# nju-ee/MODE-2022

Hardware: AMD Instinct MI355X
Metric: ERP stereo pairs/sec (512x1024, 192 disp) fwd+bwd (higher is better)
Workload: dtype fp32 storage/accumulate; products: 2xfp16 split (22-bit, per-tensor 2^k scale, 3 MFMAs) in the stride-1 3x3x3 / spherical / 3x3 layers incl. gradients (DESIGN 3u/3v); 3xbf16 split (24-bit, 6 MFMAs) in the stride-2 / transposed 3x3x3 layers and the polar spherical tiles (3j-3l); fp32 MFMA in the 32->; 1 GPU; ModeDisparity(192,Sphere,1024x512 Cassini) fwd+bwd+Adam step, batch 2/GPU (BASELINE configs[2]); global_batch=2, conv_arith=bf16x6, init=recipe state, seed 1 (tests/golden/recipe.py), parallelism=dp1

## Files before the change

mode-2022_amd/csrc/classif_head.hip:

```cpp
#include "bn_internal.h"
#include "conv3d_internal.h"

#include <algorithm>

namespace {

typedef float f32x16 __attribute__((ext_vector_type(16)));
constexpr int NT = 256;

__device__ __forceinline__ f32x16 mfma32(float a, float b, f32x16 c) { return __builtin_amdgcn_mfma_f32_32x32x2f32(a, b, c, 0, 0, 0); }

constexpr int ZTH = 16, ZIH = ZTH + 2, ZIW = 34, ZPL = ZIH * ZIW;
constexpr int ZDC = 12;
static_assert(ZIH + 2 == 4 * 5, "18 row groups + 36 halo-column positions in 2 groups = 5 groups per wave");

template <bool BNRELU, bool C32>
__global__ __launch_bounds__(NT, 2) void classif_fwd_kernel(const float* __restrict__ x, const float* __restrict__ w,
                                                            const float* __restrict__ scale, const float* __restrict__ shift,
                                                            const float* __restrict__ add, float* __restrict__ y, int B, int Ci, int D,
                                                            int H, int W, int nDc, int nHt, int nWt) {
  extern __shared__ __attribute__((aligned(16))) float zl[];
  float2* coefl = reinterpret_cast<float2*>(zl + 27 * ZPL);
  int t = xcd_remap(blockIdx.x, gridDim.x);
  const int wt = t % nWt;
  t /= nWt;
  const int ht = t % nHt;
  t /= nHt;
  const int dc = t % nDc;
  const int b = t / nDc;
  const int w0 = wt * 32, h0 = ht * ZTH, dlo = dc * ZDC, dhi = min(D, dlo + ZDC);
  const int tid = threadIdx.x, wave = tid >> 6, lane = tid & 63;
  const int j = lane & 31, kh = lane >> 5;
  const long long HW = (long long)H * W, DHW = (long long)D * HW;
  const float* xb = x + (long long)b * Ci * DHW;

  if (BNRELU && tid < 32) coefl[tid] = tid < Ci ? make_float2(scale[tid], shift[tid]) : make_float2(0.f, 0.f);
  float a0[16];
#pragma unroll
  for (int ks = 0; ks < 16; ++ks) {
    const int c = ks + 16 * kh;
    a0[ks] = (j < 27 && c < Ci) ? w[min(c, Ci - 1) * 27 + min(j, 26)] : 0.f;
  }
  int poff[5], pz[5];
  bool pok[5];
#pragma unroll
  for (int g5 = 0; g5 < 5; ++g5) {
    const int g = wave * 5 + g5;
    int row, gw, zc;
    bool in = true;
    if (g < ZIH) {
      row = g;
      gw = w0 + j;
      zc = 1 + j;
    } else {
      const int p = (g - ZIH) * 32 + j;
      in = p < 2 * ZIH;
      row = in ? p >> 1 : 0;
      gw = (p & 1) ? w0 + 32 : w0 - 1;
      zc = (p & 1) ? 33 : 0;
    }
    const int gh = h0 + row - 1;
    pok[g5] = in && gh >= 0 && gh < H && gw >= 0 && gw < W;
    poff[g5] = pok[g5] ? gh * W + gw : 0;
    pz[g5] = in ? row * ZIW + zc : -1;
  }
  if (C32) {
#pragma unroll
    for (int g5 = 0; g5 < 5; ++g5) poff[g5] += (int)((unsigned)(16 * kh) * (unsigned)DHW);
  }
  const int wx = tid & 31, hq = tid >> 5;
  float om1[2] = {0.f, 0.f}, o0[2] = {0.f, 0.f};

  float bv[5][16];
  auto load_group = [&](int dz, int g5) {
    const float* xp = xb + (long long)dz * HW;
    if (C32) {
      const unsigned pbyte = (unsigned)poff[g5] << 2;
#pragma unroll
      for (int ks = 0; ks < 16; ++ks)
        bv[g5][ks] = *reinterpret_cast<const float*>(reinterpret_cast<const char*>(xp + (long long)ks * DHW) + pbyte);
    } else {
      unsigned dhw = (unsigned)DHW;
      asm volatile("" : "+s"(dhw));
#pragma unroll
      for (int ks = 0; ks < 16; ++ks) bv[g5][ks] = xp[(unsigned)poff[g5] + (unsigned)min(ks + 16 * kh, Ci - 1) * dhw];
    }
  };
  const int dstart = max(dlo - 1, 0), dend = min(dhi, D - 1);
#pragma unroll
  for (int g5 = 0; g5 < 5; ++g5) load_group(dstart, g5);
  __syncthreads();
  const int gwx = w0 + wx;
  long long oidx[2];
  bool ook[2];
#pragma unroll
  for (int o = 0; o < 2; ++o) {
    const int gh = h0 + hq + 8 * o;
    ook[o] = gh < H && gwx < W;
    oidx[o] = ook[o] ? (long long)b * DHW + (long long)gh * W + gwx : 0;
  }

  for (int dz = dstart; dz <= dend; ++dz) {
    float s[3][2];
    const int dout = dz - 1;
    float addv[2] = {0.f, 0.f};
    if (add) {
#pragma unroll
      for (int o = 0; o < 2; ++o) addv[o] = add[oidx[o] + (long long)max(dout, 0) * HW];
    }
    f32x16 acc[5];
    int co = 16 * kh;
    const int dnext = min(dz + 1, dend);
#pragma unroll
    for (int g5 = 0; g5 < 5; ++g5) {
      asm volatile("" : "+v"(co));
      acc[g5] = (f32x16){0};
#pragma unroll
      for (int ks = 0; ks < 16; ++ks) {
        if (BNRELU) {
          const float2 cf = coefl[co + ks];
          float a = __builtin_fmaf(bv[g5][ks], cf.x, cf.y);
          asm("" : "+v"(a));
          acc[g5] = mfma32(a0[ks], pok[g5] ? relu_nan(a) : 0.f, acc[g5]);
        } else {
          acc[g5] = mfma32(a0[ks], pok[g5] ? bv[g5][ks] : 0.f, acc[g5]);
        }
      }
      __builtin_amdgcn_sched_barrier(0);
      load_group(dnext, g5);
      __builtin_amdgcn_sched_barrier(0);
    }
#pragma unroll
    for (int g5 = 0; g5 < 5; ++g5) {
      if (pz[g5] >= 0) {
#pragma unroll
        for (int q = 0; q < 16; ++q) {
          const int i = (q & 3) + 8 * (q >> 2) + 4 * kh;
          if (i < 27) zl[i * ZPL + pz[g5]] = acc[g5][q];
        }
      }
    }
    __syncthreads();
#pragma unroll
    for (int o = 0; o < 2; ++o) {
      const float* zp = zl + (hq + 8 * o) * ZIW + wx;
#pragma unroll
      for (int kd = 0; kd < 3; ++kd) {
        float v = 0.f;
#pragma unroll
        for (int k9 = 0; k9 < 9; ++k9) {
          v += zp[(kd * 9 + k9) * ZPL + (k9 / 3) * ZIW + (k9 % 3)];
          asm volatile("" : "+v"(v));
        }
        s[kd][o] = v;
      }
    }
    __syncthreads();
#pragma unroll
    for (int o = 0; o < 2; ++o) {
      if (dout >= dlo && ook[o]) y[oidx[o] + (long long)dout * HW] = om1[o] + s[2][o] + addv[o];
      om1[o] = o0[o] + s[1][o];
      o0[o] = s[0][o];
    }
  }
  if (dend < dhi) {
#pragma unroll
    for (int o = 0; o < 2; ++o) {
      if (ook[o]) {
        const long long idx = oidx[o] + (long long)dend * HW;
        y[idx] = add ? om1[o] + add[idx] : om1[o];
      }
    }
  }
}

constexpr int GTH = 8;
constexpr int XS = GTH * 32 + 1;
constexpr int GH = GTH + 2, GW = 34, GPL = GH * GW;

__global__ __launch_bounds__(NT) void classif_bww_kernel(const float* __restrict__ gy, const float* __restrict__ x,
                                                         const float* __restrict__ mean, const float* __restrict__ scale,
                                                         const float* __restrict__ shift, float* __restrict__ part, int B, int Ci, int D,
                                                         int H, int W, int nHt, int nWt, int T, int S) {
  __shared__ __attribute__((aligned(16))) float xl[32 * XS];
  __shared__ float gl[3 * GPL];
  const int s = blockIdx.x;
  const int tid = threadIdx.x, wave = tid >> 6, lane = tid & 63;
  const int hwv = tid >> 5, l32 = tid & 31;
  const long long HW = (long long)H * W, DHW = (long long)D * HW;
  const int j = lane & 31;
  const int tap = j < 27 ? j : 0;
  const int toff = (2 - tap / 9) * GPL + (2 - (tap / 3) % 3) * GW + (2 - tap % 3);
  const float mu = j < Ci ? mean[j] : 0.f, sc = j < Ci ? scale[j] : 0.f, sh = j < Ci ? shift[j] : 0.f;
  const float nanv = __builtin_nanf("");
  f32x16 accq = {0}, accm = {0};

  for (int tt = s; tt < T; tt += S) {
    int t = tt;
    const int wt = t % nWt;
    t /= nWt;
    const int ht = t % nHt;
    t /= nHt;
    const int d0 = t % D;
    const int b = t / D;
    const int w0 = wt * 32, h0 = ht * GTH;
    const float* xb = x + (long long)b * Ci * DHW + d0 * HW;
    const float* gb = gy + (long long)b * DHW;
#pragma unroll 1
    for (int kb = 0; kb < 256; kb += 64) {
      float t8[8];
#pragma unroll
      for (int jj = 0; jj < 8; ++jj) {
        const int r = kb + jj * 8 + hwv;
        const int c = r >> 3, gh = h0 + (r & 7), gw = w0 + l32;
        const bool ok = c < Ci && gh < H && gw < W;
        const float v = xb[ok ? c * DHW + (long long)gh * W + gw : 0];
        t8[jj] = ok ? v : nanv;
      }
#pragma unroll
      for (int jj = 0; jj < 8; ++jj) {
        const int r = kb + jj * 8 + hwv;
        xl[(r >> 3) * XS + (r & 7) * 32 + l32] = t8[jj];
      }
    }
    for (int idx = tid; idx < 3 * GPL; idx += NT) {
      const int zz = idx / GPL, rem = idx - zz * GPL;
      const int yy = rem / GW, xx = rem - yy * GW;
      const int gd = d0 - 1 + zz, gh = h0 - 1 + yy, gw = w0 - 1 + xx;
      const bool ok = gd >= 0 && gd < D && gh >= 0 && gh < H && gw >= 0 && gw < W;
      const float v = gb[ok ? gd * HW + (long long)gh * W + gw : 0];
      gl[idx] = ok ? v : 0.f;
    }
    __syncthreads();
    const float* ap = xl + (lane & 31) * XS + (lane >> 5);
    const float* bp = gl + toff + (lane >> 5);
#pragma unroll
    for (int rr = 0; rr < 2; ++rr) {
      const int row = wave * 2 + rr;
#pragma unroll 8
      for (int ks = 0; ks < 16; ++ks) {
        const float yv = ap[row * 32 + 2 * ks], gv = bp[row * GW + 2 * ks];
        const bool m = __builtin_fmaf(yv, sc, sh) > 0.f;
        accq = mfma32(m ? yv - mu : 0.f, gv, accq);
        accm = mfma32(m ? 1.f : 0.f, gv, accm);
      }
    }
    __syncthreads();
  }
  float* red = xl;
#pragma unroll
  for (int q = 0; q < 16; ++q) {
    const int i = (q & 3) + 8 * (q >> 2) + 4 * (lane >> 5);
    red[wave * 1024 + i * 32 + (lane & 31)] = accq[q];
    red[4096 + wave * 1024 + i * 32 + (lane & 31)] = accm[q];
  }
  __syncthreads();
  float* pb = part + (long long)s * 2048;
  for (int idx = tid; idx < 2048; idx += NT) {
    const float* r = red + (idx >> 10) * 4096 + (idx & 1023);
    float lo = r[0] + r[1024], hi = r[2048] + r[3072];
    asm volatile("" : "+v"(lo), "+v"(hi));
    pb[idx] = lo + hi;
  }
}

constexpr int XS2 = 260;

template <int TC>
__global__ __launch_bounds__(NT) void classif_bww2_kernel(const float* __restrict__ gy, const float* __restrict__ x,
                                                          const float* __restrict__ mean, const float* __restrict__ scale,
                                                          const float* __restrict__ shift, float* __restrict__ part, int B, int Ci, int D,
                                                          int H, int W, int nHt, int nWt, int T, int S) {
  constexpr int TR = 256 / TC, GWD = TC + 2, GHT = TR + 2, GPL2 = GHT * GWD, NG = (3 * GPL2 + NT - 1) / NT;
  __shared__ __attribute__((aligned(16))) float xl[32 * XS2];
  __shared__ float gl[3 * GPL2];
  const int s = blockIdx.x;
  const int tid = threadIdx.x, wave = tid >> 6, lane = tid & 63;
  const long long HW = (long long)H * W, DHW = (long long)D * HW;
  const int j = lane & 31, khalf = lane >> 5;
  const int tap = j < 27 ? j : 0;
  const int toff = (2 - tap / 9) * GPL2 + (2 - (tap / 3) % 3) * GWD + (2 - tap % 3);
  const float mu = j < Ci ? mean[j] : 0.f, sc = j < Ci ? scale[j] : 0.f, sh = j < Ci ? shift[j] : 0.f;
  const float nanv = __builtin_nanf("");
  f32x16 accq = {0}, accm = {0};

  const int v0 = 4 * (tid & 63), srow = v0 / TC, scol = v0 % TC;
  float4 px[8];
  float pg[NG];
  unsigned pxok = 0, pgok = 0;
  auto request = [&](int tt) {
    int t = tt;
    const int wt = t % nWt;
    t /= nWt;
    const int ht = t % nHt;
    t /= nHt;
    const int d0 = t % D;
    const int b = t / D;
    const int w0 = wt * TC, h0 = ht * TR;
    const float* xb = x + (long long)b * Ci * DHW + d0 * HW;
    const float* gb = gy + (long long)b * DHW;
    const int gh = h0 + srow, gw = w0 + scol;
    const unsigned vok = (unsigned)(gh < H) & (unsigned)(gw < W);
    const long long voff = (long long)vok * ((long long)gh * W + gw);
    pxok = 0;
#pragma unroll
    for (int i = 0; i < 8; ++i) {
      const int c = (tid >> 6) + 4 * i;
      px[i] = *reinterpret_cast<const float4*>(xb + (long long)min(c, Ci - 1) * DHW + voff);
      pxok |= (vok & (unsigned)(c < Ci)) << i;
    }
    pgok = 0;
#pragma unroll
    for (int i = 0; i < NG; ++i) {
      const int idx = min(tid + NT * i, 3 * GPL2 - 1);
      const int zz = idx / GPL2, rem = idx - zz * GPL2;
      const int yy = rem / GWD, xx = rem - yy * GWD;
      const int gd = d0 - 1 + zz, gh2 = h0 - 1 + yy, gw2 = w0 - 1 + xx;
      const unsigned ok = (unsigned)(gd >= 0) & (unsigned)(gd < D) & (unsigned)(gh2 >= 0) & (unsigned)(gh2 < H) & (unsigned)(gw2 >= 0) &
                          (unsigned)(gw2 < W);
      pg[i] = gb[(long long)ok * (gd * HW + (long long)gh2 * W + gw2)];
      pgok |= ok << i;
    }
  };
  if (s < T) request(s);
  asm volatile("s_waitcnt vmcnt(0)" ::: "memory");

  for (int tt = s; tt < T; tt += S) {
    __syncthreads();
#pragma unroll
    for (int i = 0; i < 8; ++i) {
      const int c = (tid >> 6) + 4 * i;
      const bool ok = (pxok >> i) & 1;
      *reinterpret_cast<float4*>(xl + c * XS2 + v0) = ok ? px[i] : make_float4(nanv, nanv, nanv, nanv);
    }
#pragma unroll
    for (int i = 0; i < NG; ++i)
      if (tid + NT * i < 3 * GPL2) gl[tid + NT * i] = ((pgok >> i) & 1) ? pg[i] : 0.f;
    __syncthreads();
    request(tt + S < T ? tt + S : tt);
    __builtin_amdgcn_sched_barrier(0);
    const float* ap = xl + j * XS2 + wave * 64 + 4 * khalf;
#pragma unroll
    for (int m = 0; m < 8; ++m) {
      const float4 a4 = *reinterpret_cast<const float4*>(ap + 8 * m);
      const int v = wave * 64 + 8 * m;
      const float* bp = gl + toff + (v / TC) * GWD + (v % TC) + 4 * khalf;
      const float ye[4] = {a4.x, a4.y, a4.z, a4.w};
#pragma unroll
      for (int e = 0; e < 4; ++e) {
        const float gv = bp[e];
        const bool mk = __builtin_fmaf(ye[e], sc, sh) > 0.f;
        accq = mfma32(mk ? ye[e] - mu : 0.f, gv, accq);
        accm = mfma32(mk ? 1.f : 0.f, gv, accm);
      }
    }
  }
  __syncthreads();
  float* red = xl;
#pragma unroll
  for (int q = 0; q < 16; ++q) {
    const int i = (q & 3) + 8 * (q >> 2) + 4 * khalf;
    red[wave * 1024 + i * 32 + j] = accq[q];
    red[4096 + wave * 1024 + i * 32 + j] = accm[q];
  }
  __syncthreads();
  float* pb = part + (long long)s * 2048;
  for (int idx = tid; idx < 2048; idx += NT) {
    const float* r = red + (idx >> 10) * 4096 + (idx & 1023);
    float lo = r[0] + r[1024], hi = r[2048] + r[3072];
    asm volatile("" : "+v"(lo), "+v"(hi));
    pb[idx] = lo + hi;
  }
}

__global__ __launch_bounds__(NT) void classif_bwd_reduce_kernel(const float* __restrict__ part, const float* __restrict__ w,
                                                                const float* __restrict__ gamma, const float* __restrict__ beta,
                                                                const float* __restrict__ mean, const float* __restrict__ invstd,
                                                                const float* __restrict__ scale, float* __restrict__ gw,
                                                                float* __restrict__ ggamma, float* __restrict__ gbeta,
                                                                float4* __restrict__ coef, int S, double count, int accumulate) {
  __shared__ double qs[27], ms[27];
  const int c = blockIdx.x, wave = threadIdx.x >> 6, lane = threadIdx.x & 63;
  for (int t = wave; t < 27; t += NT / 64) {
    const float* p = part + c * 32 + t;
    double q = 0.0, m = 0.0;
    for (int s = lane; s < S; s += 64) {
      q += (double)p[(long long)s * 2048];
      m += (double)p[(long long)s * 2048 + 1024];
    }
#pragma unroll
    for (int off = 32; off > 0; off >>= 1) {
      q += __shfl_xor(q, off, 64);
      m += __shfl_xor(m, off, 64);
    }
    if (lane == 0) {
      qs[t] = q;
      ms[t] = m;
    }
  }
  __syncthreads();
  if (threadIdx.x < 27) {
    const int t = threadIdx.x;
    const float v = (float)((double)scale[c] * qs[t] + (double)beta[c] * ms[t]);
    gw[c * 27 + t] = accumulate ? gw[c * 27 + t] + v : v;
  }
  if (threadIdx.x == 0) {
    double sgy = 0.0, sg = 0.0;
    for (int t = 0; t < 27; ++t) {
      sgy += (double)w[c * 27 + t] * qs[t];
      sg += (double)w[c * 27 + t] * ms[t];
    }
    const double is = invstd[c], mu = mean[c], gm = gamma[c];
    const double dgamma = is * sgy;
    const double A = gm * is;
    coef[c] = make_float4((float)A, (float)(-A * is * dgamma / count), (float)(A * (mu * is * dgamma - sg) / count), 0.f);
    if (accumulate) {
      ggamma[c] += (float)dgamma;
      gbeta[c] += (float)sg;
    } else {
      ggamma[c] = (float)dgamma;
      gbeta[c] = (float)sg;
    }
  }
}

constexpr int BTD = 2, BTH = 8;
constexpr int BID = BTD + 2, BIH = BTH + 2, BIW = 34;

__global__ __launch_bounds__(NT) void classif_bwd_apply_kernel(const float* __restrict__ gy, const float* __restrict__ w,
                                                               const float* __restrict__ y, const float* __restrict__ scale,
                                                               const float* __restrict__ shift, const float4* __restrict__ coef,
                                                               float* __restrict__ gx, int B, int Ci, int D, int H, int W, int nDt,
                                                               int nHt, int nWt) {
  __shared__ float tile[BID * BIH * BIW];
  __shared__ __attribute__((aligned(16))) float ctab[32 * 8];
  int t = xcd_remap(blockIdx.x, gridDim.x);
  const int wt = t % nWt;
  t /= nWt;
  const int ht = t % nHt;
  t /= nHt;
  const int dt = t % nDt;
  const int b = t / nDt;
  const int w0 = wt * 32, h0 = ht * BTH, d0 = dt * BTD;
  const int tid = threadIdx.x, wave = tid >> 6, lane = tid & 63;
  const long long HW = (long long)H * W, DHW = (long long)D * HW;
  const float* gb = gy + (long long)b * DHW;

  for (int idx = tid; idx < BID * BIH * BIW; idx += NT) {
    const int dz = idx / (BIH * BIW), rem = idx - dz * (BIH * BIW);
    const int hy = rem / BIW, wx = rem - hy * BIW;
    const int gd = d0 + dz - 1, gh = h0 + hy - 1, gw = w0 + wx - 1;
    const bool ok = gd >= 0 && gd < D && gh >= 0 && gh < H && gw >= 0 && gw < W;
    const float v = gb[ok ? gd * HW + gh * W + gw : 0];
    tile[idx] = ok ? v : 0.f;
  }
  if (tid < 32) {
    const int c = tid < Ci ? tid : Ci - 1;
    const float4 k = coef[c];
    ctab[tid * 8 + 0] = scale[c];
    ctab[tid * 8 + 1] = shift[c];
    ctab[tid * 8 + 2] = k.x;
    ctab[tid * 8 + 3] = k.y;
    ctab[tid * 8 + 4] = k.z;
  }
  float a[14];
  int toff[14];
  const int c = lane & 31;
#pragma unroll
  for (int ks = 0; ks < 14; ++ks) {
    const int k = 2 * ks + (lane >> 5);
    a[ks] = (k < 27 && c < Ci) ? w[c * 27 + 26 - k] : 0.f;
    const int kk = k < 27 ? k : 26;
    toff[ks] = (kk / 9) * (BIH * BIW) + ((kk / 3) % 3) * BIW + kk % 3;
  }
  const int gw = w0 + (lane & 31);
  long long sp[4];
  bool rok[4];
#pragma unroll
  for (int r = 0; r < 4; ++r) {
    const int row = wave * 4 + r;
    const int gd = d0 + row / BTH, gh = h0 + row % BTH;
    rok[r] = gd < D && gh < H && gw < W;
    sp[r] = rok[r] ? gd * HW + (long long)gh * W + gw : 0;
  }
  __syncthreads();

  f32x16 acc[4];
#pragma unroll
  for (int r = 0; r < 4; ++r) acc[r] = (f32x16){0};
  const float* tp = tile + (lane & 31);
#pragma unroll
  for (int ks = 0; ks < 14; ++ks)
#pragma unroll
    for (int r = 0; r < 4; ++r) {
      const int row = wave * 4 + r;
      acc[r] = mfma32(a[ks], tp[(row / BTH) * (BIH * BIW) + (row % BTH) * BIW + toff[ks]], acc[r]);
    }

  const float* yb = y + (long long)b * Ci * DHW;
  float* gxb = gx + (long long)b * Ci * DHW;
#pragma unroll
  for (int q = 0; q < 16; ++q) {
    const int i = (q & 3) + 8 * (q >> 2) + 4 * (lane >> 5);
    const int ic = i < Ci ? i : Ci - 1;
    const float4 k0 = *reinterpret_cast<const float4*>(ctab + ic * 8);
    const float Cc = ctab[ic * 8 + 4];
    float yv[4];
// ... 266 lines not shown
```

mode-2022_amd/csrc/conv1x1.hip:

```cpp
#include "common.h"

namespace {

typedef float f32x16 __attribute__((ext_vector_type(16)));
constexpr int NT = 256;

__device__ __forceinline__ f32x16 mfma32(float a, float b, f32x16 c) {
  return __builtin_amdgcn_mfma_f32_32x32x2f32(a, b, c, 0, 0, 0);
}

struct P1 {
  int B, K, rows;
  int H, W, Ho, Wo;
  int s;
  int NK4;
  int MT;
};

__global__ void pack_w1(const float* __restrict__ w, float* __restrict__ wp, int rows, int K, int MT, int NK4, int flip, int fold,
                        mode_bn_epilogue bn) {
  const long long total = (long long)MT * NK4 * 64 * 4;
  if (fold && blockIdx.x == 0)
    for (int o = threadIdx.x; o < rows; o += blockDim.x) wp[total + o] = fold_shift(bn, o);
  for (long long idx = (long long)blockIdx.x * blockDim.x + threadIdx.x; idx < total; idx += (long long)gridDim.x * blockDim.x) {
    const int j = (int)(idx & 3);
    const int lane = (int)((idx >> 2) & 63);
    const long long r = idx >> 8;
    const int k4 = (int)(r % NK4), mt = (int)(r / NK4);
    const int o = mt * 32 + (lane & 31), c = 8 * k4 + 2 * j + (lane >> 5);
    float v = 0.f;
    if (o < rows && c < K) v = flip ? w[(long long)c * rows + o] : w[(long long)o * K + c];
    if (fold && o < rows) v *= fold_scale(bn, o);
    wp[idx] = v;
  }
}

template <int MTB, bool EPI, bool SCATTER>
__global__ __launch_bounds__(NT) void conv1x1_kernel(const float* __restrict__ x, const float4* __restrict__ wp, float* __restrict__ y,
                                                     P1 d, Epi epi) {
  const int wave = threadIdx.x >> 6, lane = threadIdx.x & 63;
  const int No = d.Ho * d.Wo;
  const int tpi = (No + 31) / 32;
  const long long tile = (long long)blockIdx.x * 4 + wave;
  if (tile >= (long long)d.B * tpi) return;
  const int b = (int)(tile / tpi);
  const int q = (int)(tile % tpi) * 32 + (lane & 31);
  const bool ok = q < No;
  const int ho = q / d.Wo, wo = q - ho * d.Wo;
  const long long kplane = SCATTER ? (long long)No : (long long)d.H * d.W;
  const long long koff = !ok ? 0 : (SCATTER ? (long long)q : (long long)ho * d.s * d.W + (long long)wo * d.s);
  const float* xb = x + (long long)b * d.K * kplane + koff;
  const int half = lane >> 5;
  const int mt0 = blockIdx.y * MTB;

  f32x16 acc[MTB];
#pragma unroll
  for (int m = 0; m < MTB; ++m) acc[m] = (f32x16){0};
  const float4* wq = wp + ((long long)mt0 * d.NK4) * 64 + lane;
  const int kmax = d.K - 1;

  float bv[4];
  float4 av[MTB];
  auto load = [&](int k4, float (&b4)[4], float4 (&a4)[MTB]) {
#pragma unroll
    for (int j = 0; j < 4; ++j) {
      const int c = min(8 * k4 + 2 * j + half, kmax);
      b4[j] = xb[(long long)c * kplane];
    }
#pragma unroll
    for (int m = 0; m < MTB; ++m) a4[m] = (mt0 + m < d.MT) ? wq[((long long)m * d.NK4 + k4) * 64] : make_float4(0.f, 0.f, 0.f, 0.f);
  };
  load(0, bv, av);
  for (int k4 = 0; k4 < d.NK4; ++k4) {
    float bn_[4];
    float4 an_[MTB];
    if (k4 + 1 < d.NK4) load(k4 + 1, bn_, an_);
    __builtin_amdgcn_sched_barrier(0);
#pragma unroll
    for (int j = 0; j < 4; ++j)
#pragma unroll
      for (int m = 0; m < MTB; ++m) {
        const float a = j == 0 ? av[m].x : j == 1 ? av[m].y : j == 2 ? av[m].z : av[m].w;
        acc[m] = mfma32(a, bv[j], acc[m]);
      }
    if (k4 + 1 < d.NK4) {
#pragma unroll
      for (int j = 0; j < 4; ++j) bv[j] = bn_[j];
#pragma unroll
      for (int m = 0; m < MTB; ++m) av[m] = an_[m];
    }
  }

  if (!ok) return;
  const long long oplane = SCATTER ? (long long)d.H * d.W : (long long)No;
  const long long ooff = SCATTER ? (long long)ho * d.s * d.W + (long long)wo * d.s : (long long)q;
  float* yb = y + (long long)b * d.rows * oplane + ooff;
#pragma unroll
  for (int m = 0; m < MTB; ++m)
#pragma unroll
    for (int r = 0; r < 16; ++r) {
      const int o = (mt0 + m) * 32 + (r & 3) + 8 * (r >> 2) + 4 * half;
      if (o < d.rows) {
        const long long idx = (long long)o * oplane;
        yb[idx] = EPI ? apply_epi(epi, acc[m][r], o, (yb - y) + idx) : acc[m][r];
      }
    }
}

template <bool EPI, bool SCATTER>
int launch1(const float* x, const float* wpack, float* y, const P1& d, hipStream_t st, const Epi& epi, const char* who) {
  const long long tiles = (long long)d.B * mode::cdiv(d.Ho * d.Wo, 32);
  const int gx = mode::cdiv(tiles, 4);
  const float4* wp4 = reinterpret_cast<const float4*>(wpack);
  if (d.MT == 1)
    hipLaunchKernelGGL((conv1x1_kernel<1, EPI, SCATTER>), dim3(gx, 1), dim3(NT), 0, st, x, wp4, y, d, epi);
  else if (d.MT == 2)
    hipLaunchKernelGGL((conv1x1_kernel<2, EPI, SCATTER>), dim3(gx, 1), dim3(NT), 0, st, x, wp4, y, d, epi);
  else
    hipLaunchKernelGGL((conv1x1_kernel<4, EPI, SCATTER>), dim3(gx, mode::cdiv(d.MT, 4)), dim3(NT), 0, st, x, wp4, y, d, epi);
  return mode::check_launch(who);
}

int check1(const void* a, const void* b, const void* c, const void* wp, int B, int Ci, int H, int W, int Co, int stride, const char* who) {
  MODE_REQUIRE(B >= 0 && Ci > 0 && Co > 0 && H > 0 && W > 0, MODE_ERR_BAD_ARG, "%s: non-positive size", who);
  MODE_REQUIRE(stride == 1 || stride == 2, MODE_ERR_UNSUPPORTED, "%s: stride %d not implemented (1 or 2)", who, stride);
  MODE_REQUIRE((long long)std::max(Ci, Co) * H * W < (1ll << 31), MODE_ERR_UNSUPPORTED, "%s: a sample larger than 2^31 elements", who);
  if (B == 0) return MODE_OK;
  MODE_REQUIRE(a && b && c && wp, MODE_ERR_BAD_ARG, "%s: null pointer", who);
  return MODE_OK;
}

int fwd1(const float* x, const float* w, float* y, float* wpack, int B, int Ci, int H, int W, int Co, int stride, hipStream_t st,
         const mode_bn_epilogue* bn, const char* who) {
  P1 d;
  d.B = B; d.K = Ci; d.rows = Co; d.H = H; d.W = W; d.s = stride;
  d.Ho = (H - 1) / stride + 1; d.Wo = (W - 1) / stride + 1;
  d.NK4 = mode::cdiv(Ci, 8); d.MT = mode::cdiv(Co, 32);
  const long long npack = (long long)d.MT * d.NK4 * 256;
  if (mode::pack_needed()) hipLaunchKernelGGL(pack_w1, dim3(mode::cdiv(npack, 256)), dim3(256), 0, st, w, wpack, Co, Ci, d.MT, d.NK4, 0, bn ? 1 : 0,
                     bn ? *bn : mode_bn_epilogue());
  const Epi epi = make_epi(bn, wpack + npack);
  return bn ? launch1<true, false>(x, wpack, y, d, st, epi, who) : launch1<false, false>(x, wpack, y, d, st, epi, who);
}

struct W1 {
  int B, Ci, Co, H, W, Ho, Wo, s;
  int groups;
  int S;
};

constexpr int BW_PX = 64;
constexpr int BW_PITCH = BW_PX + 1;
constexpr int BW_TILE = 128 * BW_PITCH;
constexpr int BW_LDS_FLOATS = 2 * BW_TILE > 3 * 4 * 1024 ? 2 * BW_TILE : 3 * 4 * 1024;

template <int S2>
__global__ __launch_bounds__(NT) void conv1x1_bww_kernel(const float* __restrict__ gy, const float* __restrict__ x, float* __restrict__ part,
                                                         W1 d) {
  extern __shared__ __attribute__((aligned(16))) float sm[];
  const int wave = threadIdx.x >> 6, lane = threadIdx.x & 63;
  const int row = lane & 31, half = lane >> 5;
  const int o0 = blockIdx.y * 64, c0 = blockIdx.z * 64;
  const long long No = (long long)d.Ho * d.Wo, HW = (long long)d.H * d.W;
  const int tiles_img = (int)((No + BW_PX - 1) / BW_PX);
  const long long total = (long long)d.B * tiles_img;
  const long long per = (total + d.S - 1) / d.S;
  const long long t_lo = (long long)blockIdx.x * per, t_hi = min(total, t_lo + per);

  const int sr = threadIdx.x >> 4, sp = (threadIdx.x & 15) * 4;
  float4 v[8];
  auto issue = [&](long long t) {
    const int b = (int)(t / tiles_img);
    const long long q = (t % tiles_img) * BW_PX + sp;
    const bool ok = q < No;
#pragma unroll
    for (int u = 0; u < 8; ++u) {
      const int r = sr + 16 * u;
      if (r < 64) {
        const int o = o0 + r;
        v[u] = *reinterpret_cast<const float4*>(gy + ((long long)b * d.Co + (o < d.Co ? o : 0)) * No + (ok ? q : 0));
        if (!ok || o >= d.Co) v[u] = make_float4(0.f, 0.f, 0.f, 0.f);
      } else {
        const int c = c0 + r - 64;
        const float* xr = x + ((long long)b * d.Ci + (c < d.Ci ? c : 0)) * HW;
        if (S2 == 1) {
          v[u] = *reinterpret_cast<const float4*>(xr + (ok ? q : 0));
        } else {
          const int ho = (int)((ok ? q : 0) / d.Wo), wo = (int)((ok ? q : 0) - (long long)ho * d.Wo);
          const float* p = xr + (long long)ho * 2 * d.W + 2 * wo;
          const float4 u0 = *reinterpret_cast<const float4*>(p), u1 = *reinterpret_cast<const float4*>(p + 4);
          v[u] = make_float4(u0.x, u0.z, u1.x, u1.z);
        }
        if (!ok || c >= d.Ci) v[u] = make_float4(0.f, 0.f, 0.f, 0.f);
      }
    }
  };
  auto commit = [&](float* buf) {
#pragma unroll
    for (int u = 0; u < 8; ++u) {
      float* p = buf + (sr + 16 * u) * BW_PITCH + sp;
      p[0] = v[u].x;
      p[1] = v[u].y;
      p[2] = v[u].z;
      p[3] = v[u].w;
    }
  };

  f32x16 acc[2][2];
#pragma unroll
  for (int i = 0; i < 4; ++i) acc[i >> 1][i & 1] = (f32x16){0};
  if (t_lo < t_hi) {
    issue(t_lo);
    commit(sm);
  }
  __syncthreads();
  int buf = 0;
  for (long long t = t_lo; t < t_hi; ++t) {
    const bool more = t + 1 < t_hi;
    if (more) issue(t + 1);
    __builtin_amdgcn_sched_barrier(0);
    const float* gt = sm + buf * BW_TILE + row * BW_PITCH + wave * 16 + half;
    const float* xt = gt + 64 * BW_PITCH;
#pragma unroll
    for (int ks = 0; ks < 8; ++ks) {
      const float a0 = gt[2 * ks], a1 = gt[32 * BW_PITCH + 2 * ks];
      const float b0 = xt[2 * ks], b1 = xt[32 * BW_PITCH + 2 * ks];
      acc[0][0] = mfma32(a0, b0, acc[0][0]);
      acc[0][1] = mfma32(a0, b1, acc[0][1]);
      acc[1][0] = mfma32(a1, b0, acc[1][0]);
      acc[1][1] = mfma32(a1, b1, acc[1][1]);
    }
    if (more) commit(sm + (buf ^ 1) * BW_TILE);
    __syncthreads();
    buf ^= 1;
  }
  float (*red)[4][1024] = reinterpret_cast<float (*)[4][1024]>(sm);
  if (wave > 0) {
#pragma unroll
    for (int t = 0; t < 4; ++t)
#pragma unroll
      for (int r = 0; r < 16; ++r) red[wave - 1][t][r * 64 + lane] = acc[t >> 1][t & 1][r];
  }
  __syncthreads();
  if (wave == 0) {
    float* pb = part + (long long)blockIdx.x * d.Co * d.Ci;
#pragma unroll
    for (int t = 0; t < 4; ++t)
#pragma unroll
      for (int r = 0; r < 16; ++r) {
        float v2 = acc[t >> 1][t & 1][r];
        v2 += red[0][t][r * 64 + lane];
        v2 += red[1][t][r * 64 + lane];
        v2 += red[2][t][r * 64 + lane];
        const int o = o0 + (t >> 1) * 32 + (r & 3) + 8 * (r >> 2) + 4 * half;
        const int c = c0 + (t & 1) * 32 + row;
        if (o < d.Co && c < d.Ci) pb[(long long)o * d.Ci + c] = v2;
      }
  }
}

int bww_splits(int B, int groups, int Co, int Ci) {
  const long long blocks = (long long)mode::cdiv(Co, 64) * mode::cdiv(Ci, 64);
  long long S = (4LL * kNumCU + blocks - 1) / blocks;
  const long long total = (long long)B * mode::cdiv(groups, 16);
  if (S > (total + 3) / 4) S = (total + 3) / 4;
  return (int)std::max(1LL, S);
}

}

extern "C" size_t mode_conv1x1_wpack_bytes(int Ci, int Co) {
  if (Ci <= 0 || Co <= 0) return 0;
  const size_t f = (size_t)mode::cdiv(Co, 32) * mode::cdiv(Ci, 8) * 256, b = (size_t)mode::cdiv(Ci, 32) * mode::cdiv(Co, 8) * 256;
  return ((f > b ? f : b) + (size_t)(Co > Ci ? Co : Ci)) * sizeof(float);
}

extern "C" int mode_conv1x1_fwd(const float* x, const float* w, float* y, float* wpack, int B, int Ci, int H, int W, int Co, int stride,
                                mode_stream_t stream) {
  const char* who = "mode_conv1x1_fwd";
  int rc = check1(x, w, y, wpack, B, Ci, H, W, Co, stride, who);
  if (rc != MODE_OK || B == 0) return rc;
  return fwd1(x, w, y, wpack, B, Ci, H, W, Co, stride, mode::as_stream(stream), nullptr, who);
}

extern "C" int mode_conv1x1_fwd_bn(const float* x, const float* w, const mode_bn_epilogue* bn, float* y, float* wpack, int B, int Ci, int H,
                                   int W, int Co, int stride, mode_stream_t stream) {
  const char* who = "mode_conv1x1_fwd_bn";
  int rc = check1(x, w, y, wpack, B, Ci, H, W, Co, stride, who);
  if (rc == MODE_OK) rc = mode::check_bn(bn, who);
  if (rc != MODE_OK || B == 0) return rc;
  return fwd1(x, w, y, wpack, B, Ci, H, W, Co, stride, mode::as_stream(stream), bn, who);
}

extern "C" int mode_conv1x1_bwd_data(const float* gy, const float* w, float* gx, float* wpack, int B, int Ci, int H, int W, int Co,
                                     int stride, mode_stream_t stream) {
  const char* who = "mode_conv1x1_bwd_data";
  int rc = check1(gy, w, gx, wpack, B, Ci, H, W, Co, stride, who);
  if (rc != MODE_OK || B == 0) return rc;
  hipStream_t st = mode::as_stream(stream);
  P1 d;
  d.B = B; d.K = Co; d.rows = Ci; d.H = H; d.W = W; d.s = stride;
  d.Ho = (H - 1) / stride + 1; d.Wo = (W - 1) / stride + 1;
  d.NK4 = mode::cdiv(Co, 8); d.MT = mode::cdiv(Ci, 32);
  const long long npack = (long long)d.MT * d.NK4 * 256;
  if (mode::pack_needed()) hipLaunchKernelGGL(pack_w1, dim3(mode::cdiv(npack, 256)), dim3(256), 0, st, w, wpack, Ci, Co, d.MT, d.NK4, 1, 0, mode_bn_epilogue());
  const Epi none = make_epi(nullptr, nullptr);
  if (stride == 1) {
    return launch1<false, false>(gy, wpack, gx, d, st, none, who);
  }
  rc = mode::zero_floats(gx, (size_t)B * Ci * H * W, st, who);
  if (rc != MODE_OK) return rc;
  return launch1<false, true>(gy, wpack, gx, d, st, none, who);
}

extern "C" size_t mode_conv1x1_bwd_weight_workspace_bytes(int B, int Ci, int H, int W, int Co, int stride) {
  if (B <= 0 || Ci <= 0 || Co <= 0 || H <= 0 || W <= 0 || stride < 1) return 0;
  const int Ho = (H - 1) / stride + 1, Wo = (W - 1) / stride + 1;
  return (size_t)bww_splits(B, Ho * Wo / 4, Co, Ci) * Co * Ci * sizeof(float);
}

extern "C" int mode_conv1x1_bwd_weight(const float* gy, const float* x, float* gw, float* workspace, int B, int Ci, int H, int W, int Co,
                                       int stride, int accumulate, mode_stream_t stream) {
  const char* who = "mode_conv1x1_bwd_weight";
  int rc = check1(gy, x, gw, workspace, B, Ci, H, W, Co, stride, who);
  if (rc != MODE_OK) return rc;
  W1 d;
  d.B = B; d.Ci = Ci; d.Co = Co; d.H = H; d.W = W; d.s = stride;
  d.Ho = (H - 1) / stride + 1; d.Wo = (W - 1) / stride + 1;
  MODE_REQUIRE(d.Wo % 4 == 0 && (stride == 1 || W % 8 == 0), MODE_ERR_UNSUPPORTED,
               "%s: needs an output width divisible by 4 (stride 2: input width divisible by 8), got %dx%d stride %d", who, H, W, stride);
  MODE_REQUIRE(((size_t)gy % 16) == 0 && ((size_t)x % 16) == 0, MODE_ERR_UNSUPPORTED, "%s: tensors must be 16-byte aligned", who);
  hipStream_t st = mode::as_stream(stream);
  if (B == 0) {
    if (!accumulate) return mode::zero_floats(gw, (size_t)Co * Ci, st, who);
    return MODE_OK;
  }
  d.groups = d.Ho * d.Wo / 4;
  d.S = bww_splits(B, d.groups, Co, Ci);
  const dim3 grid(d.S, mode::cdiv(Co, 64), mode::cdiv(Ci, 64));
  const size_t lds = (size_t)BW_LDS_FLOATS * sizeof(float);
  rc = stride == 1 ? mode::allow_lds(conv1x1_bww_kernel<1>, lds, who) : mode::allow_lds(conv1x1_bww_kernel<2>, lds, who);
  if (rc != MODE_OK) return rc;
  if (stride == 1)
    hipLaunchKernelGGL(conv1x1_bww_kernel<1>, grid, dim3(NT), lds, st, gy, x, workspace, d);
  else
    hipLaunchKernelGGL(conv1x1_bww_kernel<2>, grid, dim3(NT), lds, st, gy, x, workspace, d);
  const int n = Co * Ci;
  hipLaunchKernelGGL(reduce_slices_kernel, dim3(mode::cdiv(n, 4)), dim3(256), 0, st, workspace, gw, n, d.S, accumulate);
  return mode::check_launch(who);
}
```

Baseline: 36.56 pairs/s.

## Switch 1x1 convs and classif head from fp32 MFMA to 3xbf16 split MFMAs

Replaces fp32 32x32x2 MFMAs in the 1x1 conv forward/bwd-data/bwd-weight kernels and the classification head (forward and BN-backward reduction) with 3-way bf16 splits using 6 bf16 MFMAs per product. Weights are pre-split at pack time into three bf16 planes, staged through double-buffered LDS in conv1x1, and the bwd-weight kernel stores split bf16 planes in LDS with a reworked pipeline. The intent is to use the much higher bf16 MFMA throughput at near-fp32 accuracy, at the cost of extra split arithmetic, more LDS traffic and register pressure, and changed numerics.

```diff
diff --git a/mode-2022_amd/csrc/classif_head.hip b/mode-2022_amd/csrc/classif_head.hip
--- a/mode-2022_amd/csrc/classif_head.hip
+++ b/mode-2022_amd/csrc/classif_head.hip
@@ -1,5 +1,6 @@
 #include "bn_internal.h"
 #include "conv3d_internal.h"
+#include "split_arith.h"
 
 #include <algorithm>
 
@@ -9,6 +10,30 @@
 constexpr int NT = 256;
 
 __device__ __forceinline__ f32x16 mfma32(float a, float b, f32x16 c) { return __builtin_amdgcn_mfma_f32_32x32x2f32(a, b, c, 0, 0, 0); }
+
+using mode::split::mfma_bf16;
+using mode::split::pack2;
+using mode::split::split3_bf16_pinned;
+
+struct Pieces {
+  uint4 p1, p2, p3;
+};
+__device__ __forceinline__ Pieces split8(const float (&v)[8]) {
+  Pieces r;
+  split3_bf16_pinned(v[0], v[1], r.p1.x, r.p2.x, r.p3.x);
+  split3_bf16_pinned(v[2], v[3], r.p1.y, r.p2.y, r.p3.y);
+  split3_bf16_pinned(v[4], v[5], r.p1.z, r.p2.z, r.p3.z);
+  split3_bf16_pinned(v[6], v[7], r.p1.w, r.p2.w, r.p3.w);
+  return r;
+}
+__device__ __forceinline__ f32x16 split6(const Pieces& a, const Pieces& b, f32x16 c) {
+  c = mfma_bf16(a.p3, b.p1, c);
+  c = mfma_bf16(a.p1, b.p3, c);
+  c = mfma_bf16(a.p2, b.p2, c);
+  c = mfma_bf16(a.p2, b.p1, c);
+  c = mfma_bf16(a.p1, b.p2, c);
+  return mfma_bf16(a.p1, b.p1, c);
+}
 
 constexpr int ZTH = 16, ZIH = ZTH + 2, ZIW = 34, ZPL = ZIH * ZIW;
 constexpr int ZDC = 12;
@@ -35,11 +60,16 @@
   const float* xb = x + (long long)b * Ci * DHW;
 
   if (BNRELU && tid < 32) coefl[tid] = tid < Ci ? make_float2(scale[tid], shift[tid]) : make_float2(0.f, 0.f);
-  float a0[16];
-#pragma unroll
-  for (int ks = 0; ks < 16; ++ks) {
-    const int c = ks + 16 * kh;
-    a0[ks] = (j < 27 && c < Ci) ? w[min(c, Ci - 1) * 27 + min(j, 26)] : 0.f;
+  Pieces wa[2];
+#pragma unroll
+  for (int s = 0; s < 2; ++s) {
+    float a0[8];
+#pragma unroll
+    for (int e = 0; e < 8; ++e) {
+      const int c = 8 * s + e + 16 * kh;
+      a0[e] = (j < 27 && c < Ci) ? w[min(c, Ci - 1) * 27 + min(j, 26)] : 0.f;
+    }
+    wa[s] = split8(a0);
   }
   int poff[5], pz[5];
   bool pok[5];
@@ -116,15 +146,21 @@
       asm volatile("" : "+v"(co));
       acc[g5] = (f32x16){0};
 #pragma unroll
-      for (int ks = 0; ks < 16; ++ks) {
-        if (BNRELU) {
-          const float2 cf = coefl[co + ks];
-          float a = __builtin_fmaf(bv[g5][ks], cf.x, cf.y);
-          asm("" : "+v"(a));
-          acc[g5] = mfma32(a0[ks], pok[g5] ? relu_nan(a) : 0.f, acc[g5]);
-        } else {
-          acc[g5] = mfma32(a0[ks], pok[g5] ? bv[g5][ks] : 0.f, acc[g5]);
+      for (int s = 0; s < 2; ++s) {
+        float av[8];
+#pragma unroll
+        for (int e = 0; e < 8; ++e) {
+          const int ks = 8 * s + e;
+          if (BNRELU) {
+            const float2 cf = coefl[co + ks];
+            float a = __builtin_fmaf(bv[g5][ks], cf.x, cf.y);
+            asm("" : "+v"(a));
+            av[e] = pok[g5] ? relu_nan(a) : 0.f;
+          } else {
+            av[e] = pok[g5] ? bv[g5][ks] : 0.f;
+          }
         }
+        acc[g5] = split6(wa[s], split8(av), acc[g5]);
       }
       __builtin_amdgcn_sched_barrier(0);
       load_group(dnext, g5);
@@ -339,20 +375,29 @@
     __syncthreads();
     request(tt + S < T ? tt + S : tt);
     __builtin_amdgcn_sched_barrier(0);
-    const float* ap = xl + j * XS2 + wave * 64 + 4 * khalf;
-#pragma unroll
-    for (int m = 0; m < 8; ++m) {
-      const float4 a4 = *reinterpret_cast<const float4*>(ap + 8 * m);
-      const int v = wave * 64 + 8 * m;
-      const float* bp = gl + toff + (v / TC) * GWD + (v % TC) + 4 * khalf;
-      const float ye[4] = {a4.x, a4.y, a4.z, a4.w};
-#pragma unroll
-      for (int e = 0; e < 4; ++e) {
-        const float gv = bp[e];
-        const bool mk = __builtin_fmaf(ye[e], sc, sh) > 0.f;
-        accq = mfma32(mk ? ye[e] - mu : 0.f, gv, accq);
-        accm = mfma32(mk ? 1.f : 0.f, gv, accm);
+    const float* ap = xl + j * XS2 + wave * 64 + 8 * khalf;
+#pragma unroll
+    for (int ks = 0; ks < 4; ++ks) {
+      const float4 alo = *reinterpret_cast<const float4*>(ap + 16 * ks), ahi = *reinterpret_cast<const float4*>(ap + 16 * ks + 4);
+      const int v = wave * 64 + 16 * ks;
+      const float* bp = gl + toff + (v / TC) * GWD + (v % TC) + 8 * khalf;
+      const float ye[8] = {alo.x, alo.y, alo.z, alo.w, ahi.x, ahi.y, ahi.z, ahi.w};
+      float qv[8], mv[8], gv[8];
+#pragma unroll
+      for (int e = 0; e < 8; ++e) {
+        gv[e] = bp[e];
+        float pre = __builtin_fmaf(ye[e], sc, sh), dy = ye[e] - mu;
+        asm("" : "+v"(pre), "+v"(dy));
+        const bool mk = pre > 0.f;
+        qv[e] = mk ? dy : 0.f;
+        mv[e] = mk ? 1.f : 0.f;
       }
+      const Pieces g = split8(gv);
+      accq = split6(split8(qv), g, accq);
+      const uint4 m1 = make_uint4(pack2(mv[0], mv[1]), pack2(mv[2], mv[3]), pack2(mv[4], mv[5]), pack2(mv[6], mv[7]));
+      accm = mfma_bf16(m1, g.p3, accm);
+      accm = mfma_bf16(m1, g.p2, accm);
+      accm = mfma_bf16(m1, g.p1, accm);
     }
   }
   __syncthreads();
diff --git a/mode-2022_amd/csrc/conv1x1.hip b/mode-2022_amd/csrc/conv1x1.hip
--- a/mode-2022_amd/csrc/conv1x1.hip
+++ b/mode-2022_amd/csrc/conv1x1.hip
@@ -1,54 +1,72 @@
 #include "common.h"
+#include "split_arith.h"
 
 namespace {
 
 typedef float f32x16 __attribute__((ext_vector_type(16)));
 constexpr int NT = 256;
 
-__device__ __forceinline__ f32x16 mfma32(float a, float b, f32x16 c) {
-  return __builtin_amdgcn_mfma_f32_32x32x2f32(a, b, c, 0, 0, 0);
-}
+using mode::split::mfma_bf16;
+using mode::split::split3_bf16_pinned;
 
 struct P1 {
   int B, K, rows;
   int H, W, Ho, Wo;
   int s;
-  int NK4;
+  int NK16;
   int MT;
 };
 
-__global__ void pack_w1(const float* __restrict__ w, float* __restrict__ wp, int rows, int K, int MT, int NK4, int flip, int fold,
+__global__ void pack_w1(const float* __restrict__ w, float* __restrict__ wp, int rows, int K, int MT, int NK16, int flip, int fold,
                         mode_bn_epilogue bn) {
-  const long long total = (long long)MT * NK4 * 64 * 4;
+  const long long nlane = (long long)MT * NK16 * 64, total = nlane * 12;
   if (fold && blockIdx.x == 0)
     for (int o = threadIdx.x; o < rows; o += blockDim.x) wp[total + o] = fold_shift(bn, o);
-  for (long long idx = (long long)blockIdx.x * blockDim.x + threadIdx.x; idx < total; idx += (long long)gridDim.x * blockDim.x) {
-    const int j = (int)(idx & 3);
-    const int lane = (int)((idx >> 2) & 63);
-    const long long r = idx >> 8;
-    const int k4 = (int)(r % NK4), mt = (int)(r / NK4);
-    const int o = mt * 32 + (lane & 31), c = 8 * k4 + 2 * j + (lane >> 5);
-    float v = 0.f;
-    if (o < rows && c < K) v = flip ? w[(long long)c * rows + o] : w[(long long)o * K + c];
-    if (fold && o < rows) v *= fold_scale(bn, o);
-    wp[idx] = v;
+  uint4* wp4 = reinterpret_cast<uint4*>(wp);
+  for (long long idx = (long long)blockIdx.x * blockDim.x + threadIdx.x; idx < nlane; idx += (long long)gridDim.x * blockDim.x) {
+    const int lane = (int)(idx & 63);
+    const long long r = idx >> 6;
+    const int k16 = (int)(r % NK16), mt = (int)(r / NK16);
+    const int o = mt * 32 + (lane & 31), c0 = 16 * k16 + 8 * (lane >> 5);
+    const float sc = (fold && o < rows) ? fold_scale(bn, o) : 1.f;
+    float v[8];
+#pragma unroll
+    for (int e = 0; e < 8; ++e) {
+      const int c = c0 + e;
+      v[e] = 0.f;
+      if (o < rows && c < K) v[e] = flip ? w[(long long)c * rows + o] : w[(long long)o * K + c];
+      if (fold) v[e] *= sc;
+    }
+    uint4 p1, p2, p3;
+    split3_bf16_pinned(v[0], v[1], p1.x, p2.x, p3.x);
+    split3_bf16_pinned(v[2], v[3], p1.y, p2.y, p3.y);
+    split3_bf16_pinned(v[4], v[5], p1.z, p2.z, p3.z);
+    split3_bf16_pinned(v[6], v[7], p1.w, p2.w, p3.w);
+    wp4[(r * 3 + 0) * 64 + lane] = p1;
+    wp4[(r * 3 + 1) * 64 + lane] = p2;
+    wp4[(r * 3 + 2) * 64 + lane] = p3;
   }
 }
 
 template <int MTB, bool EPI, bool SCATTER>
-__global__ __launch_bounds__(NT) void conv1x1_kernel(const float* __restrict__ x, const float4* __restrict__ wp, float* __restrict__ y,
+__global__ __launch_bounds__(NT) void conv1x1_kernel(const float* __restrict__ x, const uint4* __restrict__ wp, float* __restrict__ y,
                                                      P1 d, Epi epi) {
+  constexpr int NA = MTB * 3 * 64;
+  constexpr int NST = (NA + NT - 1) / NT;
+  __shared__ uint4 al[2][NA];
   const int wave = threadIdx.x >> 6, lane = threadIdx.x & 63;
   const int No = d.Ho * d.Wo;
   const int tpi = (No + 31) / 32;
-  const long long tile = (long long)blockIdx.x * 4 + wave;
-  if (tile >= (long long)d.B * tpi) return;
+  const long long ntile = (long long)d.B * tpi;
+  const long long tile_ = (long long)blockIdx.x * 4 + wave;
+  const bool live = tile_ < ntile;
+  const long long tile = live ? tile_ : ntile - 1;
   const int b = (int)(tile / tpi);
   const int q = (int)(tile % tpi) * 32 + (lane & 31);
-  const bool ok = q < No;
+  const bool ok = live && q < No;
   const int ho = q / d.Wo, wo = q - ho * d.Wo;
   const long long kplane = SCATTER ? (long long)No : (long long)d.H * d.W;
-  const long long koff = !ok ? 0 : (SCATTER ? (long long)q : (long long)ho * d.s * d.W + (long long)wo * d.s);
+  const long long koff = q >= No ? 0 : (SCATTER ? (long long)q : (long long)ho * d.s * d.W + (long long)wo * d.s);
   const float* xb = x + (long long)b * d.K * kplane + koff;
   const int half = lane >> 5;
   const int mt0 = blockIdx.y * MTB;
@@ -56,39 +74,65 @@
   f32x16 acc[MTB];
 #pragma unroll
   for (int m = 0; m < MTB; ++m) acc[m] = (f32x16){0};
-  const float4* wq = wp + ((long long)mt0 * d.NK4) * 64 + lane;
   const int kmax = d.K - 1;
 
-  float bv[4];
-  float4 av[MTB];
-  auto load = [&](int k4, float (&b4)[4], float4 (&a4)[MTB]) {
-#pragma unroll
-    for (int j = 0; j < 4; ++j) {
-      const int c = min(8 * k4 + 2 * j + half, kmax);
-      b4[j] = xb[(long long)c * kplane];
-    }
-#pragma unroll
-    for (int m = 0; m < MTB; ++m) a4[m] = (mt0 + m < d.MT) ? wq[((long long)m * d.NK4 + k4) * 64] : make_float4(0.f, 0.f, 0.f, 0.f);
-  };
-  load(0, bv, av);
-  for (int k4 = 0; k4 < d.NK4; ++k4) {
-    float bn_[4];
-    float4 an_[MTB];
-    if (k4 + 1 < d.NK4) load(k4 + 1, bn_, an_);
+  uint4 as[NST];
+  auto a_request = [&](int k16) {
+#pragma unroll
+    for (int u = 0; u < NST; ++u) {
+      const int i = threadIdx.x + NT * u, m = i / 192;
+      const unsigned in = (unsigned)(i < NA) & (unsigned)(mt0 + m < d.MT);
+      as[u] = wp[(long long)in * (((long long)(mt0 + m) * d.NK16 + k16) * 192 + (i - m * 192))];
+      if (!in) as[u] = make_uint4(0u, 0u, 0u, 0u);
+    }
+  };
+  auto a_commit = [&](int buf) {
+#pragma unroll
+    for (int u = 0; u < NST; ++u)
+      if (threadIdx.x + NT * u < NA) al[buf][threadIdx.x + NT * u] = as[u];
+  };
+  auto b_request = [&](int k16, float (&b8)[8]) {
+#pragma unroll
+    for (int e = 0; e < 8; ++e) {
+      const int c = min(16 * k16 + 8 * half + e, kmax);
+      b8[e] = xb[(long long)c * kplane];
+    }
+  };
+  const int klast = d.NK16 - 1;
+  auto step = [&](int k16, float (&bc)[8]) {
+    a_request(min(k16 + 1, klast));
+    if (k16 > klast) {
+#pragma unroll
+      for (int e = 0; e < 8; ++e) bc[e] = 0.f;
+    }
+    uint4 b1, b2, b3;
+    split3_bf16_pinned(bc[0], bc[1], b1.x, b2.x, b3.x);
+    split3_bf16_pinned(bc[2], bc[3], b1.y, b2.y, b3.y);
+    split3_bf16_pinned(bc[4], bc[5], b1.z, b2.z, b3.z);
+    split3_bf16_pinned(bc[6], bc[7], b1.w, b2.w, b3.w);
+    b_request(min(k16 + 2, klast), bc);
     __builtin_amdgcn_sched_barrier(0);
-#pragma unroll
-    for (int j = 0; j < 4; ++j)
-#pragma unroll
-      for (int m = 0; m < MTB; ++m) {
-        const float a = j == 0 ? av[m].x : j == 1 ? av[m].y : j == 2 ? av[m].z : av[m].w;
-        acc[m] = mfma32(a, bv[j], acc[m]);
-      }
-    if (k4 + 1 < d.NK4) {
-#pragma unroll
-      for (int j = 0; j < 4; ++j) bv[j] = bn_[j];
-#pragma unroll
-      for (int m = 0; m < MTB; ++m) av[m] = an_[m];
-    }
+    const uint4* ap = al[k16 & 1] + lane;
+#define MODE_C1_TERM(PA, PB) _Pragma("unroll") for (int m = 0; m < MTB; ++m) acc[m] = mfma_bf16(ap[(m * 3 + PA) * 64], PB, acc[m]);
+    MODE_C1_TERM(2, b1)
+    MODE_C1_TERM(0, b3)
+    MODE_C1_TERM(1, b2)
+    MODE_C1_TERM(1, b1)
+    MODE_C1_TERM(0, b2)
+    MODE_C1_TERM(0, b1)
+#undef MODE_C1_TERM
+    a_commit((k16 + 1) & 1);
+    mode::split::lds_barrier();
+  };
+  float bv0[8], bv1[8];
+  a_request(0);
+  b_request(0, bv0);
+  b_request(min(1, klast), bv1);
+  a_commit(0);
+  mode::split::lds_barrier();
+  for (int k16 = 0; k16 < d.NK16; k16 += 2) {
+    step(k16, bv0);
+    step(k16 + 1, bv1);
   }
 
   if (!ok) return;
@@ -111,7 +155,7 @@
 int launch1(const float* x, const float* wpack, float* y, const P1& d, hipStream_t st, const Epi& epi, const char* who) {
   const long long tiles = (long long)d.B * mode::cdiv(d.Ho * d.Wo, 32);
   const int gx = mode::cdiv(tiles, 4);
-  const float4* wp4 = reinterpret_cast<const float4*>(wpack);
+  const uint4* wp4 = reinterpret_cast<const uint4*>(wpack);
   if (d.MT == 1)
     hipLaunchKernelGGL((conv1x1_kernel<1, EPI, SCATTER>), dim3(gx, 1), dim3(NT), 0, st, x, wp4, y, d, epi);
   else if (d.MT == 2)
@@ -135,9 +179,9 @@
   P1 d;
   d.B = B; d.K = Ci; d.rows = Co; d.H = H; d.W = W; d.s = stride;
   d.Ho = (H - 1) / stride + 1; d.Wo = (W - 1) / stride + 1;
-  d.NK4 = mode::cdiv(Ci, 8); d.MT = mode::cdiv(Co, 32);
-  const long long npack = (long long)d.MT * d.NK4 * 256;
-  if (mode::pack_needed()) hipLaunchKernelGGL(pack_w1, dim3(mode::cdiv(npack, 256)), dim3(256), 0, st, w, wpack, Co, Ci, d.MT, d.NK4, 0, bn ? 1 : 0,
+  d.NK16 = mode::cdiv(Ci, 16); d.MT = mode::cdiv(Co, 32);
+  const long long npack = (long long)d.MT * d.NK16 * 768;
+  if (mode::pack_needed()) hipLaunchKernelGGL(pack_w1, dim3(mode::cdiv(npack / 12, 256)), dim3(256), 0, st, w, wpack, Co, Ci, d.MT, d.NK16, 0, bn ? 1 : 0,
                      bn ? *bn : mode_bn_epilogue());
   const Epi epi = make_epi(bn, wpack + npack);
   return bn ? launch1<true, false>(x, wpack, y, d, st, epi, who) : launch1<false, false>(x, wpack, y, d, st, epi, who);
@@ -150,14 +194,15 @@
 };
 
 constexpr int BW_PX = 64;
-constexpr int BW_PITCH = BW_PX + 1;
-constexpr int BW_TILE = 128 * BW_PITCH;
-constexpr int BW_LDS_FLOATS = 2 * BW_TILE > 3 * 4 * 1024 ? 2 * BW_TILE : 3 * 4 * 1024;
+constexpr int BW_PITCH = 2 * BW_PX + 16;
+constexpr int BW_PLANE = 128 * BW_PITCH;
+constexpr int BW_LDS_BYTES = 3 * BW_PLANE > 3 * 4 * 1024 * 4 ? 3 * BW_PLANE : 3 * 4 * 1024 * 4;
+static_assert(BW_PITCH % 16 == 0, "16-byte fragment reads");
 
 template <int S2>
 __global__ __launch_bounds__(NT) void conv1x1_bww_kernel(const float* __restrict__ gy, const float* __restrict__ x, float* __restrict__ part,
                                                          W1 d) {
-  extern __shared__ __attribute__((aligned(16))) float sm[];
+  extern __shared__ __attribute__((aligned(16))) unsigned char sm[];
   const int wave = threadIdx.x >> 6, lane = threadIdx.x & 63;
   const int row = lane & 31, half = lane >> 5;
   const int o0 = blockIdx.y * 64, c0 = blockIdx.z * 64;
@@ -195,14 +240,16 @@
       }
     }
   };
-  auto commit = [&](float* buf) {
+  auto commit = [&]() {
 #pragma unroll
     for (int u = 0; u < 8; ++u) {
-      float* p = buf + (sr + 16 * u) * BW_PITCH + sp;
-      p[0] = v[u].x;
-      p[1] = v[u].y;
-      p[2] = v[u].z;
-      p[3] = v[u].w;
+      uint2 p1, p2, p3;
+      split3_bf16_pinned(v[u].x, v[u].y, p1.x, p2.x, p3.x);
+      split3_bf16_pinned(v[u].z, v[u].w, p1.y, p2.y, p3.y);
+      unsigned char* p = sm + (sr + 16 * u) * BW_PITCH + sp * 2;
+      *reinterpret_cast<uint2*>(p) = p1;
+      *reinterpret_cast<uint2*>(p + BW_PLANE) = p2;
+      *reinterpret_cast<uint2*>(p + 2 * BW_PLANE) = p3;
     }
   };
 
@@ -211,28 +258,38 @@
   for (int i = 0; i < 4; ++i) acc[i >> 1][i & 1] = (f32x16){0};
   if (t_lo < t_hi) {
     issue(t_lo);
-    commit(sm);
+    commit();
+    if (t_lo + 1 < t_hi) issue(t_lo + 1);
   }
   __syncthreads();
-  int buf = 0;
+  const unsigned char* gt = sm + row * BW_PITCH + (wave * 16 + half * 8) * 2;
   for (long long t = t_lo; t < t_hi; ++t) {
-    const bool more = t + 1 < t_hi;
-    if (more) issue(t + 1);
-    __builtin_amdgcn_sched_barrier(0);
-    const float* gt = sm + buf * BW_TILE + row * BW_PITCH + wave * 16 + half;
-    const float* xt = gt + 64 * BW_PITCH;
-#pragma unroll
-    for (int ks = 0; ks < 8; ++ks) {
-      const float a0 = gt[2 * ks], a1 = gt[32 * BW_PITCH + 2 * ks];
-      const float b0 = xt[2 * ks], b1 = xt[32 * BW_PITCH + 2 * ks];
-      acc[0][0] = mfma32(a0, b0, acc[0][0]);
-      acc[0][1] = mfma32(a0, b1, acc[0][1]);
-      acc[1][0] = mfma32(a1, b0, acc[1][0]);
-      acc[1][1] = mfma32(a1, b1, acc[1][1]);
-    }
-    if (more) commit(sm + (buf ^ 1) * BW_TILE);
+    uint4 a[2][3], b[2][3];
+#pragma unroll
+    for (int h = 0; h < 2; ++h)
+#pragma unroll
+      for (int p = 0; p < 3; ++p) {
+        a[h][p] = *reinterpret_cast<const uint4*>(gt + p * BW_PLANE + h * 32 * BW_PITCH);
+        b[h][p] = *reinterpret_cast<const uint4*>(gt + p * BW_PLANE + (64 + h * 32) * BW_PITCH);
+      }
     __syncthreads();
-    buf ^= 1;
+    if (t + 1 < t_hi) {
+      commit();
+      if (t + 2 < t_hi) issue(t + 2);
+    }
+#define MODE_BWW_TERM(PA, PB)                                \
+  acc[0][0] = mfma_bf16(a[0][PA], b[0][PB], acc[0][0]);      \
+  acc[0][1] = mfma_bf16(a[0][PA], b[1][PB], acc[0][1]);      \
+  acc[1][0] = mfma_bf16(a[1][PA], b[0][PB], acc[1][0]);      \
+  acc[1][1] = mfma_bf16(a[1][PA], b[1][PB], acc[1][1]);
+    MODE_BWW_TERM(2, 0)
+    MODE_BWW_TERM(0, 2)
+    MODE_BWW_TERM(1, 1)
+    MODE_BWW_TERM(1, 0)
+    MODE_BWW_TERM(0, 1)
+    MODE_BWW_TERM(0, 0)
+#undef MODE_BWW_TERM
+    __syncthreads();
   }
   float (*red)[4][1024] = reinterpret_cast<float (*)[4][1024]>(sm);
   if (wave > 0) {
@@ -271,7 +328,7 @@
 
 extern "C" size_t mode_conv1x1_wpack_bytes(int Ci, int Co) {
   if (Ci <= 0 || Co <= 0) return 0;
-  const size_t f = (size_t)mode::cdiv(Co, 32) * mode::cdiv(Ci, 8) * 256, b = (size_t)mode::cdiv(Ci, 32) * mode::cdiv(Co, 8) * 256;
+  const size_t f = (size_t)mode::cdiv(Co, 32) * mode::cdiv(Ci, 16) * 768, b = (size_t)mode::cdiv(Ci, 32) * mode::cdiv(Co, 16) * 768;
   return ((f > b ? f : b) + (size_t)(Co > Ci ? Co : Ci)) * sizeof(float);
 }
 
@@ -301,9 +358,9 @@
   P1 d;
   d.B = B; d.K = Co; d.rows = Ci; d.H = H; d.W = W; d.s = stride;
   d.Ho = (H - 1) / stride + 1; d.Wo = (W - 1) / stride + 1;
-  d.NK4 = mode::cdiv(Co, 8); d.MT = mode::cdiv(Ci, 32);
-  const long long npack = (long long)d.MT * d.NK4 * 256;
-  if (mode::pack_needed()) hipLaunchKernelGGL(pack_w1, dim3(mode::cdiv(npack, 256)), dim3(256), 0, st, w, wpack, Ci, Co, d.MT, d.NK4, 1, 0, mode_bn_epilogue());
+  d.NK16 = mode::cdiv(Co, 16); d.MT = mode::cdiv(Ci, 32);
+  const long long npack = (long long)d.MT * d.NK16 * 768;
+  if (mode::pack_needed()) hipLaunchKernelGGL(pack_w1, dim3(mode::cdiv(npack / 12, 256)), dim3(256), 0, st, w, wpack, Ci, Co, d.MT, d.NK16, 1, 0, mode_bn_epilogue());
   const Epi none = make_epi(nullptr, nullptr);
   if (stride == 1) {
     return launch1<false, false>(gy, wpack, gx, d, st, none, who);
@@ -338,7 +395,7 @@
   d.groups = d.Ho * d.Wo / 4;
   d.S = bww_splits(B, d.groups, Co, Ci);
   const dim3 grid(d.S, mode::cdiv(Co, 64), mode::cdiv(Ci, 64));
-  const size_t lds = (size_t)BW_LDS_FLOATS * sizeof(float);
+  const size_t lds = (size_t)BW_LDS_BYTES;
   rc = stride == 1 ? mode::allow_lds(conv1x1_bww_kernel<1>, lds, who) : mode::allow_lds(conv1x1_bww_kernel<2>, lds, who);
   if (rc != MODE_OK) return rc;
   if (stride == 1)
```

Result: no change. 36.76 pairs/s, median of 6 (+0.5%).
